# TrungMasterChef/CSWin-SimAM-UNet

Measured on AMD Instinct MI355X. Metric: images/sec at 512×512 bf16, 1/2/4/8 MI355X; Dice parity vs reference, higher is better.
Workload: dtype bf16; 1 GPU; CSWin-UNet train step 512x512 depth [1, 2, 9, 1] split [1, 2, 8, 8] +SimAM, AdamW; model=CSWinTransformer, params=23567980, global_batch=16, per_gpu_batch=16, img=512, parallelism=dp1, workload_key=cswin|d1,2,9,1|s1,2,8,8|simam|bf16|512|16

## Files before the change

cswin-simam-unet_amd/csrc/gemm_ws.hip:

```cpp
#include "common.hpp"

#include <type_traits>

namespace csu {
namespace {

enum { WS_PLAIN = 0, WS_RESID = 1, WS_LNBWD = 2, WS_RESID_LN = 3 };

struct WsLnF {
    const float* gamma;
    const float* beta;
    float eps;
    bf16* out;
    float* mean;
    float* rstd;
};

struct WsLn {
    const float* x;
    const float* gamma;
    const float* mean;
    const float* rstd;
    const float* dres;
    float* dx;
    bf16* dxb;
    float* part;
};

constexpr int WS_BM = 64;
constexpr bool WS_ROT = true;

constexpr int ws_unit(int ks, int nt, int umax = 16) {
    for (int u = umax; u > 1; --u)
        if (ks % u == 0 && nt * (ks / u) >= 2) return u;
    for (int u = umax; u > 1; --u)
        if (ks % u == 0) return u;
    return 1;
}
constexpr int ws_wn(int n) { return (n / 32) % 4 == 0 ? 4 : (n / 32) % 2 == 0 ? 2 : 1; }
constexpr int ws_tokens(int n) { return WS_BM * (4 / ws_wn(n)); }
#ifndef WS_NSPLIT
#define WS_NSPLIT 1
#endif
constexpr int ws_ns(int k, int n, int epi) {
    return WS_NSPLIT > 1 && epi == 0 && k <= 256 && ws_wn(n) == 4 && (n / 128) % WS_NSPLIT == 0 ? WS_NSPLIT : 1;
}

__device__ __forceinline__ bf16x8 e4m3x8_bf16(u32x2 w) {
    typedef __bf16 bf16x2v __attribute__((ext_vector_type(2)));
    const bf16x2v p0 = __builtin_amdgcn_cvt_scalef32_pk_bf16_fp8(w[0], 1.f, false);
    const bf16x2v p1 = __builtin_amdgcn_cvt_scalef32_pk_bf16_fp8(w[0], 1.f, true);
    const bf16x2v p2 = __builtin_amdgcn_cvt_scalef32_pk_bf16_fp8(w[1], 1.f, false);
    const bf16x2v p3 = __builtin_amdgcn_cvt_scalef32_pk_bf16_fp8(w[1], 1.f, true);
    return bf16x8{p0[0], p0[1], p1[0], p1[1], p2[0], p2[1], p3[0], p3[1]};
}

template <int K, int N, int EPI, typename TOUT, int NS = 1, int F8 = 0>
__global__ __launch_bounds__(256, ws_wn(N) < 4 || NS > 1 ? 2 : 1) void gemm_ws_kernel(long M, const bf16* __restrict__ X, int ldx,
                                                      const bf16* __restrict__ Wf, const float* __restrict__ bias,
                                                      const float* __restrict__ resid, TOUT* __restrict__ out,
                                                      WsLn ln = WsLn{}, WsLnF lnf = WsLnF{},
                                                      const float* __restrict__ wsc = nullptr) {
    static_assert(F8 == 0 || EPI != WS_LNBWD, "gemm_ws: e4m3 weights not with the LayerNorm-backward epilogue");
    constexpr int WN = ws_wn(N);
    constexpr int NT = N / (32 * WN * NS);
    static_assert(NT * 32 * WN * NS == N, "gemm_ws: N = 32 WN NT NS");
    static_assert(NS == 1 || EPI == WS_PLAIN || EPI == WS_RESID, "gemm_ws: the LayerNorm epilogues need all N features");
    static_assert(EPI != WS_LNBWD || WN == 4, "gemm_ws: the LayerNorm epilogue needs all C features in one token group");
    constexpr int KS = K / 16;
    constexpr int UK = ws_unit(KS, NT, NS > 1 ? 8 : 16);
    constexpr int CH = KS / UK;
    static_assert(CH * UK == KS, "unit size");
    constexpr int U = NT * CH;
    constexpr bool XREG = K <= 256;
    constexpr bool XLDS = !XREG || WN == 4;
    constexpr int XS = K + 8;
    constexpr int ES = 36;
    __shared__ __attribute__((aligned(16))) bf16 xs[XLDS ? WS_BM * XS : 8];
    __shared__ __attribute__((aligned(16))) float ep_all[4 * WS_BM * ES];

    const int lane = threadIdx.x & 63;
    const int wave = __builtin_amdgcn_readfirstlane(threadIdx.x >> 6);
    const int wn = wave % WN;
    const int r = lane & 31, h = lane >> 5;
    const long m0 = (long)blockIdx.x * ws_tokens(N) + WS_BM * (wave / WN);
    float* ep = ep_all + wave * WS_BM * ES;

    const int rot = WS_ROT ? (int)((blockIdx.x >> 3) % NT) : 0;
    const int tb = NS > 1 ? (int)blockIdx.y * NT : 0;
    auto tile_of = [&](int i) { return tb + (i + rot < NT ? i + rot : i + rot - NT); };
    using WFR = std::conditional_t<F8 != 0, u32x2, bf16x8>;
    WFR wf[2][UK];
    auto wload1 = [&](int u, int s) {
        const int nt = wn + WN * tile_of(u / CH), ks = (u % CH) * UK + s;
        if constexpr (F8 != 0)
            wf[u & 1][s] = *reinterpret_cast<const u32x2*>(reinterpret_cast<const uint8_t*>(Wf) +
                                                           ((long)(nt * KS + ks) * 64 + lane) * 8);
        else
            wf[u & 1][s] = *reinterpret_cast<const bf16x8*>(Wf + ((long)(nt * KS + ks) * 64 + lane) * 8);
    };
    auto wfrag = [&](const WFR& w) {
        if constexpr (F8 != 0) return e4m3x8_bf16(w);
        else return w;
    };
#pragma unroll
    for (int s = 0; s < UK; ++s) wload1(0, s);
    __builtin_amdgcn_sched_barrier(0);
    bf16x8 xf[XREG ? 2 : 1][XREG ? KS : 1];
    if constexpr (XLDS) {
        constexpr int PR = K / 8;
#pragma unroll
        for (int i = 0; i < WS_BM * PR / 256; ++i) {
            const int p = threadIdx.x + 256 * i, row = p / PR, c = 8 * (p % PR);
            bf16x8 v = *reinterpret_cast<const bf16x8*>(X + (m0 + row) * ldx + c);
            if constexpr (F8 == 2) {
                const f32x4 s0 = *reinterpret_cast<const f32x4*>(wsc + c), s1 = *reinterpret_cast<const f32x4*>(wsc + c + 4);
#pragma unroll
                for (int e = 0; e < 4; ++e) {
                    v[e] = (bf16)((float)v[e] * s0[e]);
                    v[4 + e] = (bf16)((float)v[4 + e] * s1[e]);
                }
            }
            *reinterpret_cast<bf16x8*>(xs + row * XS + c) = v;
        }
        __syncthreads();
        if constexpr (XREG) {
#pragma unroll
            for (int t = 0; t < 2; ++t)
#pragma unroll
                for (int s = 0; s < KS; ++s) xf[t][s] = *reinterpret_cast<const bf16x8*>(xs + (32 * t + r) * XS + 16 * s + 8 * h);
        }
    } else {
#pragma unroll
        for (int t = 0; t < 2; ++t)
#pragma unroll
            for (int s = 0; s < KS; ++s) {
                xf[t][s] = *reinterpret_cast<const bf16x8*>(X + (m0 + 32 * t + r) * ldx + 16 * s + 8 * h);
                if constexpr (F8 == 2) {
#pragma unroll
                    for (int e = 0; e < 8; ++e) xf[t][s][e] = (bf16)((float)xf[t][s][e] * wsc[16 * s + 8 * h + e]);
                }
            }
    }
    __builtin_amdgcn_sched_barrier(0);

    f32x16 a0 = f32x16{}, a1 = f32x16{};
    const auto rs_b = buf_rsrc(bias, bias ? (long)N * 4 : 0);
    constexpr bool BF = sizeof(TOUT) == 2;
    constexpr bool RES = EPI == WS_RESID || EPI == WS_RESID_LN;
    static_assert(EPI != WS_RESID_LN || !BF, "gemm_ws: the LayerNorm epilogue writes the fp32 residual stream");
    float bv[8], rv[8][4], sv[8];
    const auto rs_s = buf_rsrc(wsc, F8 == 1 ? (long)N * 4 : 0);
    f32x16 keep[EPI == WS_LNBWD ? NT : 1][2];
    float yk[EPI == WS_RESID_LN ? NT : 1][8][4];
    float lg[EPI == WS_RESID_LN ? NT : 1][4], lb[EPI == WS_RESID_LN ? NT : 1][4];
    if constexpr (EPI == WS_RESID_LN) {
        const int cc = 4 * (lane & 7);
#pragma unroll
        for (int i = 0; i < NT; ++i) {
            load4(lnf.gamma + 32 * (wn + WN * tile_of(i)) + cc, lg[i]);
            load4(lnf.beta + 32 * (wn + WN * tile_of(i)) + cc, lb[i]);
        }
    }
#pragma unroll
    for (int u = 0; u < U; ++u) {
        const int c = u % CH;
        if (EPI != WS_LNBWD && c == CH - 1) {
            const int n0 = 32 * (wn + WN * tile_of(u / CH));
            if constexpr (BF) {
                const int cc = 8 * (lane & 3);
                buf_ld4(rs_b, (unsigned)(n0 + cc) * 4, bv);
                buf_ld4(rs_b, (unsigned)(n0 + cc + 4) * 4, bv + 4);
                if constexpr (F8 == 1) {
                    buf_ld4(rs_s, (unsigned)(n0 + cc) * 4, sv);
                    buf_ld4(rs_s, (unsigned)(n0 + cc + 4) * 4, sv + 4);
                }
            } else {
                const int cc = 4 * (lane & 7);
                buf_ld4(rs_b, (unsigned)(n0 + cc) * 4, bv);
                if constexpr (F8 == 1) buf_ld4(rs_s, (unsigned)(n0 + cc) * 4, sv);
                if constexpr (RES) {
                    const auto rs_res = buf_rsrc(resid + m0 * N, (M - m0) * N * 4);
#pragma unroll
                    for (int q = 0; q < 8; ++q) buf_ld4(rs_res, (unsigned)((8 * q + (lane >> 3)) * N + n0 + cc) * 4, rv[q]);
                }
            }
        }
        __builtin_amdgcn_sched_barrier(0);
#pragma unroll
        for (int s = 0; s < UK; ++s) {
            if (u + 1 < U) wload1(u + 1, s);
            const int ks = c * UK + s;
            bf16x8 b0, b1;
            if constexpr (XREG) {
                b0 = xf[0][ks];
                b1 = xf[XREG ? 1 : 0][ks];
            } else {
                b0 = *reinterpret_cast<const bf16x8*>(xs + r * XS + 16 * ks + 8 * h);
                b1 = *reinterpret_cast<const bf16x8*>(xs + (32 + r) * XS + 16 * ks + 8 * h);
            }
            const bf16x8 wa = wfrag(wf[u & 1][s]);
            a0 = __builtin_amdgcn_mfma_f32_32x32x16_bf16(wa, b0, a0, 0, 0, 0);
            a1 = __builtin_amdgcn_mfma_f32_32x32x16_bf16(wa, b1, a1, 0, 0, 0);
            if (u + 1 < U) __builtin_amdgcn_sched_group_barrier(0x020, 1, 0);
            if constexpr (!XREG) __builtin_amdgcn_sched_group_barrier(0x100, 2, 0);
            __builtin_amdgcn_sched_group_barrier(0x008, 2, 0);
        }
        __builtin_amdgcn_sched_barrier(0);
        if (c != CH - 1) continue;
        if constexpr (EPI == WS_LNBWD) {
            keep[u / CH][0] = a0;
            keep[u / CH][1] = a1;
            a0 = f32x16{};
            a1 = f32x16{};
            continue;
        }
        const int nt = wn + WN * tile_of(u / CH);
#pragma unroll
        for (int t = 0; t < 2; ++t) {
            const f32x16& a = t ? a1 : a0;
#pragma unroll
            for (int g = 0; g < 4; ++g)
                *reinterpret_cast<f32x4*>(ep + (32 * t + r) * ES + 8 * g + 4 * h) =
                    f32x4{a[4 * g], a[4 * g + 1], a[4 * g + 2], a[4 * g + 3]};
        }
        asm volatile("" ::: "memory");
        const int n0 = 32 * nt;
        const auto rs_out = buf_rsrc(out + m0 * N, (M - m0) * N * (long)sizeof(TOUT));
        if constexpr (BF) {
            const int cc = 8 * (lane & 3);
#pragma unroll
            for (int q = 0; q < 4; ++q) {
                const int row = 16 * q + (lane >> 2);
                float v[8];
                load4(ep + row * ES + cc, v);
                load4(ep + row * ES + cc + 4, v + 4);
#pragma unroll
                for (int e = 0; e < 8; ++e) {
                    if constexpr (F8 == 1) v[e] *= sv[e];
                    v[e] += bv[e];
                }
                buf_st8bf(rs_out, (unsigned)(row * N + n0 + cc) * 2, v);
            }
        } else {
            const int cc = 4 * (lane & 7);
#pragma unroll
            for (int q = 0; q < 8; ++q) {
                const int row = 8 * q + (lane >> 3);
                float v[4];
                load4(ep + row * ES + cc, v);
#pragma unroll
                for (int e = 0; e < 4; ++e) {
                    if constexpr (F8 == 1) v[e] *= sv[e];
                    v[e] += bv[e];
                    if constexpr (RES) v[e] += rv[q][e];
                    if constexpr (EPI == WS_RESID_LN) yk[u / CH][q][e] = v[e];
                }
                buf_st4(rs_out, (unsigned)(row * N + n0 + cc) * 4, v);
            }
        }
        a0 = f32x16{};
        a1 = f32x16{};
        __builtin_amdgcn_sched_barrier(0);
    }
    if constexpr (EPI == WS_RESID_LN) {
        __shared__ float lnx[2][4][WS_BM];
        const int rq = lane >> 3, g0 = (wave / WN) * WN;
        float mu[8], rsd[8];
#pragma unroll
        for (int pass = 0; pass < 2; ++pass) {
#pragma unroll
            for (int q = 0; q < 8; ++q) {
                float a = 0.f;
#pragma unroll
                for (int i = 0; i < NT; ++i)
#pragma unroll
                    for (int e = 0; e < 4; ++e) {
                        const float d = pass ? yk[i][q][e] - mu[q] : yk[i][q][e];
                        a = pass ? fmaf(d, d, a) : a + d;
                    }
                a = sum8_dpp(a);
                if ((lane & 7) == 0) lnx[pass][wave][8 * q + rq] = a;
            }
            __syncthreads();
#pragma unroll
            for (int q = 0; q < 8; ++q) {
                float t = 0.f;
#pragma unroll
                for (int j = 0; j < WN; ++j) t += lnx[pass][g0 + j][8 * q + rq];
                if (pass) rsd[q] = rsqrtf(t * (1.f / N) + lnf.eps);
                else mu[q] = t * (1.f / N);
            }
        }
        const auto rs_ln = buf_rsrc(lnf.out + m0 * N, (M - m0) * N * 2);
        const int cc = 4 * (lane & 7);
#pragma unroll
        for (int i = 0; i < NT; ++i) {
            const int n0 = 32 * (wn + WN * tile_of(i));
#pragma unroll
            for (int q = 0; q < 8; ++q) {
                float o[4];
#pragma unroll
                for (int e = 0; e < 4; ++e) o[e] = (yk[i][q][e] - mu[q]) * rsd[q] * lg[i][e] + lb[i][e];
                buf_st4bf(rs_ln, (unsigned)((8 * q + rq) * N + n0 + cc) * 2, o);
            }
        }
        if (wn == 0 && (lane & 7) == 0) {
#pragma unroll
            for (int q = 0; q < 8; ++q) {
                lnf.mean[m0 + 8 * q + rq] = mu[q];
                lnf.rstd[m0 + 8 * q + rq] = rsd[q];
            }
        }
    }
    if constexpr (EPI == WS_LNBWD) {
        constexpr int C = N;
        const auto rs_x = buf_rsrc(ln.x + m0 * C, (M - m0) * C * 4);
        const auto rs_r = buf_rsrc(ln.dres ? ln.dres + m0 * C : nullptr, ln.dres ? (M - m0) * C * 4 : 0);
        float mu[2], rs[2];
#pragma unroll
        for (int t = 0; t < 2; ++t) {
            mu[t] = ln.mean[m0 + 32 * t + r];
            rs[t] = ln.rstd[m0 + 32 * t + r];
        }
        float xh[NT][2][16], gam[NT][16];
        float rv2[NT][2][16];
#pragma unroll
        for (int i = 0; i < NT; ++i) {
            const int n0 = 32 * (wn + WN * tile_of(i));
#pragma unroll
            for (int g = 0; g < 4; ++g) {
                load4(ln.gamma + n0 + 8 * g + 4 * h, gam[i] + 4 * g);
#pragma unroll
                for (int t = 0; t < 2; ++t) {
                    const unsigned off = (unsigned)((32 * t + r) * C + n0 + 8 * g + 4 * h) * 4;
                    buf_ld4(rs_x, off, xh[i][t] + 4 * g);
                    buf_ld4(rs_r, off, rv2[i][t] + 4 * g);
                }
            }
        }
        float s1[2] = {0.f, 0.f}, s2[2] = {0.f, 0.f};
        float dgc[NT][16], dbc[NT][16];
#pragma unroll
        for (int i = 0; i < NT; ++i)
#pragma unroll
            for (int j = 0; j < 16; ++j) {
                dgc[i][j] = 0.f;
                dbc[i][j] = 0.f;
#pragma unroll
                for (int t = 0; t < 2; ++t) {
                    const float dh = keep[i][t][j];
                    const float x_h = (xh[i][t][j] - mu[t]) * rs[t];
                    xh[i][t][j] = x_h;
                    const float gg = dh * gam[i][j];
                    s1[t] += gg;
                    s2[t] += gg * x_h;
                    dgc[i][j] += dh * x_h;
                    dbc[i][j] += dh;
                }
            }
        float* lnx = ep_all;
#pragma unroll
        for (int t = 0; t < 2; ++t) {
            s1[t] += __shfl_xor(s1[t], 32, 64);
            s2[t] += __shfl_xor(s2[t], 32, 64);
            if (h == 0) {
                lnx[(wave * 2 + 0) * 64 + 32 * t + r] = s1[t];
                lnx[(wave * 2 + 1) * 64 + 32 * t + r] = s2[t];
            }
        }
        __syncthreads();
        float S1[2], S2[2];
#pragma unroll
        for (int t = 0; t < 2; ++t) {
            S1[t] = S2[t] = 0.f;
#pragma unroll
            for (int w = 0; w < 4; ++w) {
                S1[t] += lnx[(w * 2 + 0) * 64 + 32 * t + r];
                S2[t] += lnx[(w * 2 + 1) * 64 + 32 * t + r];
            }
            S1[t] *= 1.f / C;
            S2[t] *= 1.f / C;
        }
        const auto rs_dx = buf_rsrc(ln.dx + m0 * C, (M - m0) * C * 4);
        const auto rs_dxb = buf_rsrc(ln.dxb + m0 * C, (M - m0) * C * 2);
#pragma unroll
        for (int i = 0; i < NT; ++i) {
            const int n0 = 32 * (wn + WN * tile_of(i));
#pragma unroll
            for (int t = 0; t < 2; ++t)
#pragma unroll
                for (int g = 0; g < 4; ++g) {
                    float o[4];
#pragma unroll
                    for (int e = 0; e < 4; ++e) {
                        const int j = 4 * g + e;
                        o[e] = rs[t] * (keep[i][t][j] * gam[i][j] - S1[t] - xh[i][t][j] * S2[t]) + rv2[i][t][j];
                    }
                    const unsigned off = (unsigned)((32 * t + r) * C + n0 + 8 * g + 4 * h);
                    buf_st4(rs_dx, off * 4, o);
                    buf_st4bf(rs_dxb, off * 2, o);
                }
        }
#pragma unroll
        for (int o = 1; o < 32; o <<= 1)
#pragma unroll
            for (int i = 0; i < NT; ++i)
#pragma unroll
                for (int j = 0; j < 16; ++j) {
                    dgc[i][j] += __shfl_xor(dgc[i][j], o, 64);
                    dbc[i][j] += __shfl_xor(dbc[i][j], o, 64);
                }
        if (r == 0) {
            float* prow = ln.part + (size_t)blockIdx.x * 2 * C;
#pragma unroll
            for (int i = 0; i < NT; ++i) {
                const int n0 = 32 * (wn + WN * tile_of(i));
#pragma unroll
                for (int g = 0; g < 4; ++g) {
                    store4(prow + n0 + 8 * g + 4 * h, dgc[i] + 4 * g);
                    store4(prow + C + n0 + 8 * g + 4 * h, dbc[i] + 4 * g);
                }
            }
        }
    }
}

template <int K, int N, int EPI, typename TOUT, int F8 = 0>
int ws_launch(long M, const bf16* X, int ldx, const bf16* Wf, const float* bias, const float* resid, void* out,
              hipStream_t st, const WsLn& ln = WsLn{}, const WsLnF& lnf = WsLnF{}, const float* wsc = nullptr) {
    constexpr int NS = F8 ? 1 : ws_ns(K, N, EPI);
    gemm_ws_kernel<K, N, EPI, TOUT, NS, F8><<<dim3((unsigned)(M / ws_tokens(N)), NS), 256, 0, st>>>(
        M, X, ldx, Wf, bias, resid, (TOUT*)out, ln, lnf, wsc);
    return check_launch("gemm_ws");
}

#define WS_SHAPES(X_) X_(128, 384) X_(256, 768) X_(384, 128) X_(768, 256) X_(128, 128) X_(256, 256) \
    X_(64, 192) X_(64, 64)

}

int gemm_ws_supported(long M, int N, int K, int resid, int out_dtype) {
    if (M < ws_tokens(N) || M % ws_tokens(N) || M > (1L << 30)) return 0;
    if (resid && out_dtype != CSU_F32) return 0;
    if (out_dtype != CSU_F32 && out_dtype != CSU_BF16) return 0;
#define WS_HAS(KK, NN) if (K == KK && N == NN) return 1;
    WS_SHAPES(WS_HAS)
#undef WS_HAS
    return 0;
}

int gemm_ws_run(long M, int N, int K, const bf16* X, int ldx, const bf16* Wf, const float* bias, const float* resid,
                int out_dtype, void* out, hipStream_t st) {
#define WS_GO(KK, NN)                                                                                             \
    if (K == KK && N == NN) {                                                                                     \
        if (resid) return ws_launch<KK, NN, WS_RESID, float>(M, X, ldx, Wf, bias, resid, out, st);          \
        if (out_dtype == CSU_F32) return ws_launch<KK, NN, WS_PLAIN, float>(M, X, ldx, Wf, bias, nullptr, out, st); \
        return ws_launch<KK, NN, WS_PLAIN, bf16>(M, X, ldx, Wf, bias, nullptr, out, st);                    \
    }
    WS_SHAPES(WS_GO)
#undef WS_GO
    return fail(CSU_E_ARG, "gemm_ws: shape not instantiated");
}

int gemm_ws_e4m3_run(long M, int N, int K, const bf16* X, int ldx, const uint8_t* Wq, const float* wsc, int mode,
                     const float* bias, const float* resid, int out_dtype, void* out, hipStream_t st) {
    const bf16* W = reinterpret_cast<const bf16*>(Wq);
#define WS_GO8(KK, NN, MODE)                                                                                      \
    if (K == KK && N == NN && mode == MODE) {                                                                     \
        if (resid) return ws_launch<KK, NN, WS_RESID, float, MODE>(M, X, ldx, W, bias, resid, out, st, {}, {}, wsc); \
        if (out_dtype == CSU_F32)                                                                                 \
            return ws_launch<KK, NN, WS_PLAIN, float, MODE>(M, X, ldx, W, bias, nullptr, out, st, {}, {}, wsc);   \
        return ws_launch<KK, NN, WS_PLAIN, bf16, MODE>(M, X, ldx, W, bias, nullptr, out, st, {}, {}, wsc);        \
    }
#define WS_GO8B(KK, NN) WS_GO8(KK, NN, 1) WS_GO8(KK, NN, 2)
    WS_SHAPES(WS_GO8B)
#undef WS_GO8B
#undef WS_GO8
    return fail(CSU_E_ARG, "gemm_ws_e4m3: shape not instantiated");
}

int gemm_ws_ln_supported(long M, int N, int K) {
    if (M < ws_tokens(N) || M % ws_tokens(N) || M > (1L << 30)) return 0;
    return K == N && (N == 64 || N == 128 || N == 256);
}

int gemm_ws_ln_run(long M, int N, const bf16* X, int ldx, const bf16* Wf, const float* bias, const float* resid, float* out,
                   const WsLnF& lnf, hipStream_t st, const float* wsc = nullptr) {
    if (wsc) {
        if (N == 64) return ws_launch<64, 64, WS_RESID_LN, float, 1>(M, X, ldx, Wf, bias, resid, out, st, WsLn{}, lnf, wsc);
        if (N == 128) return ws_launch<128, 128, WS_RESID_LN, float, 1>(M, X, ldx, Wf, bias, resid, out, st, WsLn{}, lnf, wsc);
        if (N == 256) return ws_launch<256, 256, WS_RESID_LN, float, 1>(M, X, ldx, Wf, bias, resid, out, st, WsLn{}, lnf, wsc);
        return fail(CSU_E_ARG, "gemm_ws_ln_e4m3: shape not instantiated");
    }
    if (N == 64) return ws_launch<64, 64, WS_RESID_LN, float>(M, X, ldx, Wf, bias, resid, out, st, WsLn{}, lnf);
    if (N == 128) return ws_launch<128, 128, WS_RESID_LN, float>(M, X, ldx, Wf, bias, resid, out, st, WsLn{}, lnf);
    if (N == 256) return ws_launch<256, 256, WS_RESID_LN, float>(M, X, ldx, Wf, bias, resid, out, st, WsLn{}, lnf);
    return fail(CSU_E_ARG, "gemm_ws_ln: shape not instantiated");
}

int gemm_ws_lnbwd_supported(long M, int N, int K) {
    if (M < WS_BM || M % WS_BM || M > (1L << 30)) return 0;
    return (K == 384 && N == 128) || (K == 768 && N == 256);
}

int gemm_ws_lnbwd_run(long M, int N, int K, const bf16* dy, const bf16* Wtf, const WsLn& ln, hipStream_t st) {
    if (K == 384 && N == 128) return ws_launch<384, 128, WS_LNBWD, float>(M, dy, K, Wtf, nullptr, nullptr, nullptr, st, ln);
    if (K == 768 && N == 256) return ws_launch<768, 256, WS_LNBWD, float>(M, dy, K, Wtf, nullptr, nullptr, nullptr, st, ln);
    return fail(CSU_E_ARG, "gemm_ws_lnbwd: shape not instantiated");
}

__global__ __launch_bounds__(256) void frag_layout_kernel(const csu_frag_item* __restrict__ items, int count) {
    const long g = (long)blockIdx.x * 256 + threadIdx.x;
    int lo = 0, hi = count - 1;
    while (lo < hi) {
        const int mid = (lo + hi + 1) >> 1;
        if (items[mid].chunk0 <= g) lo = mid; else hi = mid - 1;
    }
    const csu_frag_item it = items[lo];
    const long q = g - it.chunk0;
    const int qc = it.cols / 8;
    if (q < 0 || q >= (long)it.rows * qc) return;
    const int n = (int)(q / qc), k8 = (int)(q % qc);
    const long dst = (((long)(n >> 5) * (it.cols >> 4) + (k8 >> 1)) * 64 + (n & 31) + 32 * (k8 & 1)) * 8;
    *reinterpret_cast<u32x4*>((bf16*)it.dst + dst) = *reinterpret_cast<const u32x4*>((const bf16*)it.src + q * 8);
}

__device__ __forceinline__ long frag8_chunk(int row, int c8, int cols) {
    return ((long)(row >> 5) * (cols >> 4) + (c8 >> 1)) * 64 + (row & 31) + 32 * (c8 & 1);
}
__global__ __launch_bounds__(256) void frag8_layout_kernel(const csu_frag8_item* __restrict__ items, int count) {
    const long g = (long)blockIdx.x * 256 + threadIdx.x;
    int lo = 0, hi = count - 1;
    while (lo < hi) {
        const int mid = (lo + hi + 1) >> 1;
        if (items[mid].block0 <= g) lo = mid; else hi = mid - 1;
    }
    const csu_frag8_item it = items[lo];
    const long b = g - it.block0;
    const int kb = it.K / 8;
    if (b < 0 || b >= (long)(it.N / 8) * kb) return;
    const int n0 = 8 * (int)(b / kb), k0 = 8 * (int)(b % kb);
    const uint8_t* src = reinterpret_cast<const uint8_t*>(it.src);
    u32x2 v[8];
#pragma unroll
    for (int i = 0; i < 8; ++i) v[i] = *reinterpret_cast<const u32x2*>(src + (long)(n0 + i) * it.K + k0);
    u32x2* dst = reinterpret_cast<u32x2*>(it.dst);
    if (!it.transpose) {
#pragma unroll
        for (int i = 0; i < 8; ++i) dst[frag8_chunk(n0 + i, k0 >> 3, it.K)] = v[i];
    } else {
#pragma unroll
        for (int j = 0; j < 8; ++j) {
            unsigned lo4 = 0, hi4 = 0;
#pragma unroll
            for (int i = 0; i < 4; ++i) {
                lo4 |= ((v[i][j >> 2] >> (8 * (j & 3))) & 0xffu) << (8 * i);
                hi4 |= ((v[4 + i][j >> 2] >> (8 * (j & 3))) & 0xffu) << (8 * i);
            }
            dst[frag8_chunk(k0 + j, n0 >> 3, it.N)] = u32x2{lo4, hi4};
        }
    }
}

}

using namespace csu;

extern "C" int csu_gemm_ws_supported(long M, int N, int K, int resid, int out_dtype) {
    return gemm_ws_supported(M, N, K, resid, out_dtype);
}

extern "C" int csu_gemm_ws(long M, int N, int K, const void* x, int ldx, const void* w_frag, const float* bias,
                           const float* resid, int out_dtype, void* out, void* stream) {
    if (!x || !w_frag || !out) return fail(CSU_E_ARG, "gemm_ws: null pointer");
    if (!gemm_ws_supported(M, N, K, resid != nullptr, out_dtype)) return fail(CSU_E_ARG, "gemm_ws: unsupported shape");
// ... 63 lines not shown
```

cswin-simam-unet_amd/csu/ops.py:

```python
from __future__ import annotations

import ctypes
import os
import threading
import weakref
from typing import List, Optional, Sequence, Tuple

import torch

from . import _lib
from ._lib import CSU_BF16, CSU_F32, CsuError, check, dtype_code, lib, ptr, require_device, stream_ptr
from .ledger import esize, launch as _launch, prec_of


def _stripe_fwd_work(geom, B, esize):
    L = geom.reso * geom.reso
    nb = len(geom.branches)
    hs, ws, _ = geom.branches[0]
    N = hs * ws
    nbytes = B * L * (3 * geom.C + geom.C) * esize + nb * B * geom.heads * L * 4
    flops = B * L * nb * geom.heads * 4 * N * geom.head_dim + 18 * B * L * geom.C
    return nbytes, flops


# ... 2122 lines not shown
            self._layout_frag8(dev)
            return self.deq
        if self.lay_count:
            _launch("quant_e4m3", lambda: lib().csu_e4m3_layout_batch(ptr(self.lay_items), self.lay_count, self.lay_words,
                                                                     stream_ptr(dev)), 0, self.lay_words * 8)
        self._layout_frag8(dev)
        return self.deq

    def _layout_frag8(self, dev):
        if self.frag8_count and FP8_WS:
            n = self.frag8_blocks * 64
            _launch("quant_e4m3", lambda: lib().csu_frag8_layout_batch(ptr(self.frag8_items), self.frag8_count,
                                                                      self.frag8_blocks, stream_ptr(dev)), 0, 2 * n)


_ACTIVE_CACHE: Optional[CastCache] = None
_ACTIVE_FP8: Optional[Fp8Weights] = None


def set_cast_cache(cache: Optional[CastCache], fp8: Optional[Fp8Weights] = None):
    global _ACTIVE_CACHE, _ACTIVE_FP8
    _ACTIVE_CACHE = cache
    _ACTIVE_FP8 = fp8


def fp8_gemm(aq: torch.Tensor, sa: torch.Tensor, wq: torch.Tensor, sw: torch.Tensor,
             bias: Optional[torch.Tensor] = None) -> torch.Tensor:
    require_device(aq, wq)
    M, K = aq.shape
    N = wq.shape[0]
    if wq.shape[1] != K or sa.numel() != M or sw.numel() != N or aq.dtype != torch.uint8 or wq.dtype != torch.uint8:
        raise ValueError("fp8_gemm: shape / dtype mismatch")
    aq, wq, sa, sw = aq.contiguous(), wq.contiguous(), sa.float().contiguous(), sw.float().contiguous()
    b = None if bias is None else bias.detach().float().contiguous()
    out = torch.empty(M, N, dtype=torch.bfloat16, device=aq.device)
    _launch("fp8_gemm", lambda: lib().csu_fp8_gemm(M, N, K, ptr(aq), ptr(sa), ptr(wq), ptr(sw), ptr(b), ptr(out),
                                                   stream_ptr(aq.device)),
            2 * M * N * K, M * K + N * K + M * N * 2 + (M + N) * 4, prec="fp8")
    return out


def dequant_e4m3_rows(q: torch.Tensor, scale: torch.Tensor) -> torch.Tensor:
    require_device(q)
    rows, cols = q.shape
    out = torch.empty(rows, cols, dtype=torch.bfloat16, device=q.device)
    _launch("dequant_e4m3", lambda: lib().csu_dequant_e4m3_rows(rows, cols, ptr(q), ptr(scale), ptr(out),
                                                                stream_ptr(q.device)),
            0, rows * cols * 3 + rows * 4, prec="fp8")
    return out


def layer_norm_fp8(x: torch.Tensor, weight: torch.Tensor, bias: torch.Tensor, eps: float = 1e-5, dq: bool = False):
    require_device(x, weight, bias)
    x = x.contiguous()
    C = x.shape[-1]
    rows = x.numel() // C
    w = weight.detach().float().contiguous()
    b = bias.detach().float().contiguous()
    q = torch.empty(rows, C, dtype=torch.uint8, device=x.device)
    s = torch.empty(rows, dtype=torch.float32, device=x.device)
    mean = torch.empty(rows, dtype=torch.float32, device=x.device)
    rstd = torch.empty(rows, dtype=torch.float32, device=x.device)
    ydq = torch.empty(rows, C, dtype=torch.bfloat16, device=x.device) if dq else None
    _launch("layernorm_fwd_fp8", lambda: lib().csu_layernorm_fwd_fp8_dq(rows, C, float(eps), dtype_code(x), ptr(x),
                                                                        ptr(w), ptr(b), ptr(q), ptr(s), ptr(ydq),
                                                                        ptr(mean), ptr(rstd), stream_ptr(x.device)),
            10 * rows * C, rows * C * (esize(x) + 1 + (2 if dq else 0)) + rows * 12, prec=prec_of(x))
    return (q, s, mean, rstd, ydq) if dq else (q, s, mean, rstd)


class _LnLinearFp8Fn(torch.autograd.Function):

    @staticmethod
    def forward(ctx, x, gamma, beta, weight, bias, eps: float, wq, ws, wt):
        x = x.contiguous()
        C = x.shape[-1]
        hq, hs, mean, rstd, hdq = layer_norm_fp8(x, gamma, beta, eps, dq=True)
        y = fp8_gemm(hq, hs, wq, ws, bias).view(*x.shape[:-1], wq.shape[0])
        ctx.save_for_backward(x, gamma.detach().float().contiguous(), mean, rstd, hdq, wt)
        ctx.params = (gamma, beta)
        ctx.pdtypes = (gamma.dtype, beta.dtype)
        ctx.lin = (weight, bias)
        ctx.lmeta = (weight.dtype, None if bias is None else bias.dtype, C)
        _note_use(ctx, gamma, beta, weight, bias)
        return x.view_as(x), y

    @staticmethod
    def backward(ctx, dres, dy):
        x, g, mean, rstd, h, wt = ctx.saved_tensors
        wdt, bdt, C = ctx.lmeta
        dh = dw = db = None
        if dy is not None:
            N = dy.shape[-1]
            dy2 = _bf16_of(dy).reshape(-1, N).contiguous()
            dh = gemm(dy2, wt, False, torch.bfloat16).view(x.shape)
            need_w, need_b = ctx.needs_input_grad[3], bdt is not None and ctx.needs_input_grad[4]
            if need_w or need_b:
                dwf, dbf = wgrad_maybe_side(dy2, h, wdt if need_w else None, bdt if need_b else None, params=ctx.lin)
                dw = dwf.to(wdt) if need_w else None
                db = dbf.to(bdt) if need_b else None
        dx, dg, dbeta = _ln_fork_backward(ctx, x, g, mean, rstd, dres, dh)
        return dx, dg, dbeta, dw, db, None, None, None, None


class _LnLinearWsFn(torch.autograd.Function):

    @staticmethod
    def forward(ctx, x, gamma, beta, weight, bias, eps: float, wf, wtf, pre):
        x = x.contiguous()
        C = x.shape[-1]
        rows = x.numel() // C
        g = gamma.detach().float().contiguous()
        if pre is not None:
            h1, mean, rstd = pre[3].view(x.shape), pre[4], pre[5]
        else:
            b = beta.detach().float().contiguous()
            h1 = torch.empty(x.shape, dtype=torch.bfloat16, device=x.device)
            mean = torch.empty(rows, dtype=torch.float32, device=x.device)
            rstd = torch.empty(rows, dtype=torch.float32, device=x.device)
            _launch("layernorm_fwd", lambda: lib().csu_layernorm_fwd(rows, C, float(eps), dtype_code(x), ptr(x), ptr(g),
                                                                     ptr(b), CSU_BF16, ptr(h1), ptr(mean), ptr(rstd),
                                                                     stream_ptr(x.device)),
                    8 * rows * C, rows * C * (4 + 2) + rows * 8, prec="f32")
        N = weight.shape[0]
        h2 = h1.view(rows, C)
        y = gemm_ws(h2, wf, N, torch.bfloat16, bias=None if bias is None else bias.detach().float().contiguous())
        ctx.save_for_backward(x, g, mean, rstd, h2, wtf)
        ctx.params = (gamma, beta)
        ctx.pdtypes = (gamma.dtype, beta.dtype)
        ctx.lin = (weight, bias)
        ctx.lmeta = (weight.dtype, None if bias is None else bias.dtype)
        _note_use(ctx, gamma, beta, weight, bias)
        return x.view_as(x), y.view(*x.shape[:-1], N)

    @staticmethod
    def backward(ctx, dres, dy):
        x, g, mean, rstd, h, wtf = ctx.saved_tensors
        wdt, bdt = ctx.lmeta
        C = x.shape[-1]
        rows = x.numel() // C
        if dy is None:
            dx, dg, dbeta = _ln_fork_backward(ctx, x, g, mean, rstd, dres, None)
            return dx, dg, dbeta, None, None, None, None, None, None
        N = dy.shape[-1]
        dy2 = _bf16_of(dy).reshape(-1, N).contiguous()
        dres_k = dres.float().contiguous() if dres is not None else None
        dx = torch.empty_like(x)
        dxb = torch.empty(x.shape, dtype=torch.bfloat16, device=x.device)
        nblk = rows // 64
        work = torch.empty(nblk * 2 * C, dtype=torch.float32, device=x.device)
        _launch("gemm", lambda: lib().csu_gemm_ws_lnbwd(rows, C, N, ptr(dy2), ptr(wtf), ptr(x), ptr(g), ptr(mean), ptr(rstd),
                                                       ptr(dres_k), ptr(dx), ptr(dxb), ptr(work), stream_ptr(x.device)),
                2 * rows * N * C + 12 * rows * C,
                rows * N * 2 + N * C * 2 + rows * C * (4 + (4 if dres_k is not None else 0) + 4 + 2) + rows * 8,
                prec="bf16", tag=f"{rows}x{C}x{N}:lnbwd:ws")
        dgb = _grad_dest(ctx.params)
        if dgb is None:
            dgb = torch.empty(2 * C, dtype=torch.float32, device=x.device)
        if not _ln_params(ctx, rows, C, work, dgb, nblocks=nblk):
            it = (_lib.LnParamItem * 1)()
            it[0].workspace, it[0].dgamma, it[0].dbeta = work.data_ptr(), dgb.data_ptr(), dgb.data_ptr() + C * 4
            it[0].rows, it[0].C, it[0].nblocks = rows, C, nblk
            _launch("layernorm_bwd", lambda: lib().csu_layernorm_param_reduce_batch(it, 1, stream_ptr(x.device)),
                    0, work.numel() * 4 + 2 * C * 4)
        dw = db = None
        need_w, need_b = ctx.needs_input_grad[3], bdt is not None and ctx.needs_input_grad[4]
        if need_w or need_b:
            dwf, dbf = wgrad_maybe_side(dy2, h, wdt if need_w else None, bdt if need_b else None, params=ctx.lin)
            dw = dwf.to(wdt) if need_w else None
            db = dbf.to(bdt) if need_b else None
        dx._csu_bf16 = dxb
        return dx, dgb[:C].to(ctx.pdtypes[0]), dgb[C:].to(ctx.pdtypes[1]), dw, db, None, None, None, None


FUSE_LN_QKV = False


def ln_linear_ws(x: torch.Tensor, ln: torch.nn.LayerNorm, lin: torch.nn.Linear):
    if not (FUSE_LN_QKV and USE_GEMM_WS and x.is_cuda and x.dtype == torch.float32 and _ACTIVE_CACHE is not None
            and (_ACTIVE_FP8 is None or not FP8_WS)):
        return None
    N, K = lin.weight.shape
    if x.shape[-1] != K or ln.weight.numel() != K or ln.weight.dtype != torch.float32:
        return None
    wf, wtf = _ACTIVE_CACHE.get_frag(lin.weight), _ACTIVE_CACHE.get_frag_t(lin.weight)
    M = x.numel() // K
    if wf is None or wtf is None or not _ws_ok(M, N, K, torch.bfloat16) or not lib().csu_gemm_ws_lnbwd_supported(M, K, N):
        return None
    pre = _ln_pre(x, ln.weight, ln.bias, ln.eps, torch.bfloat16)
    with torch.autocast("cuda", enabled=False):
        return _LnLinearWsFn.apply(x, ln.weight, ln.bias, lin.weight, lin.bias, ln.eps, wf, wtf, pre)


FP8_QKV = os.environ.get("CSU_FP8_QKV", "0") != "0"


def ln_linear_fp8(x: torch.Tensor, ln: torch.nn.LayerNorm, lin: torch.nn.Linear):
    if _ACTIVE_FP8 is None or not x.is_cuda or not FP8_QKV:
        return None
    got = _ACTIVE_FP8.lookup(lin.weight)
    N, K = lin.weight.shape
    if got is None or N % 64 or K % 64 or K > 512:
        return None
    wc = _ACTIVE_CACHE.get(lin.weight, torch.bfloat16) if _ACTIVE_CACHE is not None else None
    if wc is None:
        return None
    wt = _weight_t(lin.weight, wc)
    with torch.autocast("cuda", enabled=False):
        return _LnLinearFp8Fn.apply(x, ln.weight, ln.bias, lin.weight, lin.bias, ln.eps, got[0], got[1], wt)


def linear(x: torch.Tensor, weight: torch.Tensor, bias: Optional[torch.Tensor] = None,
           out_dtype: Optional[torch.dtype] = None) -> torch.Tensor:
    if x.is_cuda and torch.is_autocast_enabled("cuda"):
        cd = torch.get_autocast_dtype("cuda")
    else:
        cd = torch.promote_types(x.dtype, weight.dtype)
    wc = _ACTIVE_CACHE.get(weight, cd) if _ACTIVE_CACHE is not None else None
    with torch.autocast("cuda", enabled=False):
        return _LinearFn.apply(x, weight, bias, cd, wc, out_dtype)


def _conv_geom(B, H, W, C, N, KH, KW, stride, pad):
    g = _lib.ConvGeom()
    g.B, g.H, g.W, g.C, g.N, g.KH, g.KW, g.stride, g.pad = B, H, W, C, N, KH, KW, stride, pad
    g.OH, g.OW = (H + 2 * pad - KH) // stride + 1, (W + 2 * pad - KW) // stride + 1
    return g


def _conv_wgrad(g, x, dy, dt, c_real=None, out=None):
    L = lib()
    cr = g.C if c_real is None else c_real
    if out is None:
        out = torch.empty(g.N * g.KH * g.KW * cr + g.N, dtype=torch.float32, device=x.device)
    n = L.csu_conv2d_wgrad_workspace(ctypes.byref(g))
    work = torch.empty(max(n, 16), dtype=torch.uint8, device=x.device)
    _launch("conv_wgrad", lambda: L.csu_conv2d_wgrad_oihw(ctypes.byref(g), dt, ptr(x), ptr(dy), cr, ptr(out), ptr(work),
                                                          n, stream_ptr(x.device)),
            2 * g.B * g.OH * g.OW * g.N * g.KH * g.KW * g.C,
            (g.B * g.H * g.W * g.C + g.B * g.OH * g.OW * g.N) * x.element_size() + out.numel() * 4, prec=prec_of(x))
    k = g.N * g.KH * g.KW * cr
    return out[:k].view(g.N, cr, g.KH, g.KW), out[k:]


def _pad_channels(C: int) -> int:
    return (C + 7) // 8 * 8 if (C % 8 and PAD_CHANNELS) else C


def _conv_ws(op: int, g, t: torch.Tensor):
    n = lib().csu_conv2d_workspace(op, ctypes.byref(g), dtype_code(t))
    if not n:
        return None, 0
    return torch.empty(n, dtype=torch.uint8, device=t.device), n


class _Conv2dFn(torch.autograd.Function):
    @staticmethod
    def forward(ctx, x, weight, bias, stride: int, pad: int, cd):
        require_device(x, weight)
        B, H, W, C = x.shape
        N, Cw, KH, KW = weight.shape
        if Cw != C:
            raise ValueError(f"conv2d: input has {C} channels, weight expects {Cw}")
        cp = _pad_channels(C)
        if cp != C:
            xn = x.permute(0, 3, 1, 2)
            if cd == torch.bfloat16 and x.dtype == torch.float32 and xn.is_contiguous():
                xc = torch.empty(B, H, W, cp, dtype=cd, device=x.device)
                _launch("pack_nhwc", lambda: lib().csu_pack_nhwc_bf16(B, C, H, W, cp, ptr(xn), ptr(xc), stream_ptr(x.device)),
                        0, x.numel() * 4 + xc.numel() * 2, prec="f32")
            else:
                xc = torch.zeros(B, H, W, cp, dtype=cd, device=x.device)
                xc[..., :C] = x
            cached = _ACTIVE_CACHE.get_conv(weight, cd) if _ACTIVE_CACHE is not None else None
            if cached is not None and cached[0].shape[-1] == cp:
                w_ohwi = cached[0]
            else:
                w_ohwi = torch.nn.functional.pad(weight.detach().permute(0, 2, 3, 1).to(cd), (0, cp - C)).contiguous()
            cached = None
        else:
            xc = (x if x.dtype == cd else x.to(cd)).contiguous()
            cached = _ACTIVE_CACHE.get_conv(weight, cd) if _ACTIVE_CACHE is not None else None
            w_ohwi = cached[0] if cached else weight.detach().permute(0, 2, 3, 1).to(cd).contiguous()
        g = _conv_geom(B, H, W, cp, N, KH, KW, stride, pad)
        y = torch.empty(B, g.OH, g.OW, N, dtype=cd, device=x.device)
        bf = None if bias is None else bias.detach().float().contiguous()
        ws, nws = _conv_ws(0, g, xc)
        _launch("conv_fwd", lambda: lib().csu_conv2d_fwd_ws(ctypes.byref(g), dtype_code(xc), ptr(xc), ptr(w_ohwi), ptr(bf),
                                                            ptr(y), ptr(ws), nws, stream_ptr(x.device)),
                2 * y.numel() * KH * KW * cp, (xc.numel() + w_ohwi.numel() + y.numel()) * xc.element_size(), prec=prec_of(xc))
        ctx.save_for_backward(xc, weight)
        ctx.w_ihwo = cached[1] if cached else None
        ctx.bias = bias
        _note_use(ctx, weight, bias)
        ctx.conf = (stride, pad, cd, x.dtype, bias is not None, None if bias is None else bias.dtype)
        return y

    @staticmethod
    def backward(ctx, dy):
        xc, weight = ctx.saved_tensors
        stride, pad, cd, xdt, has_b, bdt = ctx.conf
        B, H, W, cp = xc.shape
        N, C, KH, KW = weight.shape
        g = _conv_geom(B, H, W, cp, N, KH, KW, stride, pad)
        dy = dy.to(cd).contiguous()
        dx = None
        if ctx.needs_input_grad[0]:
            if cp != C:
                w_ihwo = torch.nn.functional.pad(weight.detach().permute(1, 2, 3, 0).to(cd), (0, 0, 0, 0, 0, 0, 0, cp - C))
                w_ihwo = w_ihwo.contiguous()
            else:
                w_ihwo = ctx.w_ihwo if ctx.w_ihwo is not None else weight.detach().permute(1, 2, 3, 0).to(cd).contiguous()
            dx = torch.empty(B, H, W, cp, dtype=cd, device=dy.device)
            ws, nws = _conv_ws(1, g, dy)
            _launch("conv_dgrad", lambda: lib().csu_conv2d_dgrad_ws(ctypes.byref(g), dtype_code(dy), ptr(dy), ptr(w_ihwo),
                                                                    None, ptr(dx), ptr(ws), nws, stream_ptr(dy.device)),
                    2 * dy.numel() * KH * KW * cp, (dy.numel() + w_ihwo.numel() + dx.numel()) * dy.element_size(),
                    prec=prec_of(dy))
            if cp != C:
                dx = dx[..., :C]
            if dx.dtype != xdt:
                dx = dx.to(xdt)

        dest = None
        if has_b and weight.dtype == torch.float32 and bdt == torch.float32:
            dest = _grad_dest((weight, ctx.bias))
            if dest is not None and dest.numel() != N * KH * KW * C + N:
                dest = None
# ... 148 lines not shown
```

Baseline: 1570 images/sec.

## Restructure LayerNorm-backward GEMM epilogue via LDS row phase and enable LN-QKV fusion

The LayerNorm-backward epilogue of the weight-stationary GEMM now writes each accumulated dh tile to shared memory instead of holding all tiles in registers. A row-wise phase then computes the normalization backward with DPP/readlane reductions, prefetching x and the residual gradient during the MFMA loop. Column partials for dgamma/dbeta are reduced through the reused token panel. Occupancy is raised to 2 for C<=128, and the fused LN+QKV path is enabled by default via an environment flag. This lowers register pressure and turns on a previously disabled fusion, at the cost of extra LDS traffic and synchronisation.

```diff
diff --git a/cswin-simam-unet_amd/csrc/gemm_ws.hip b/cswin-simam-unet_amd/csrc/gemm_ws.hip
--- a/cswin-simam-unet_amd/csrc/gemm_ws.hip
+++ b/cswin-simam-unet_amd/csrc/gemm_ws.hip
@@ -55,8 +55,27 @@
     return bf16x8{p0[0], p0[1], p1[0], p1[1], p2[0], p2[1], p3[0], p3[1]};
 }
 
+template <int LPR> __device__ __forceinline__ float ln_row_sum(float x) {
+    x = sum8_dpp(x);
+    x += dppf<0x128>(x);
+    x = xsum16(x);
+    if constexpr (LPR == 64) x = xsum32(x);
+    return x;
+}
+template <int RPI> __device__ __forceinline__ float ln_row_val(float v, int i, int lane) {
+    const int b = __builtin_bit_cast(int, v);
+    if constexpr (RPI == 1) return __builtin_bit_cast(float, __builtin_amdgcn_readlane(b, i));
+    else {
+        const int lo = __builtin_amdgcn_readlane(b, 2 * i), hi = __builtin_amdgcn_readlane(b, 2 * i + 1);
+        return __builtin_bit_cast(float, lane < 32 ? lo : hi);
+    }
+}
+
+constexpr int ws_ep_floats(int n, int epi) { return epi == WS_LNBWD ? WS_BM * (n + 4) / 2 : 4 * WS_BM * 36; }
+constexpr int ws_occ(int n, int epi, int ns) { return ws_wn(n) < 4 || ns > 1 || (epi == WS_LNBWD && n <= 128) ? 2 : 1; }
+
 template <int K, int N, int EPI, typename TOUT, int NS = 1, int F8 = 0>
-__global__ __launch_bounds__(256, ws_wn(N) < 4 || NS > 1 ? 2 : 1) void gemm_ws_kernel(long M, const bf16* __restrict__ X, int ldx,
+__global__ __launch_bounds__(256, ws_occ(N, EPI, NS)) void gemm_ws_kernel(long M, const bf16* __restrict__ X, int ldx,
                                                       const bf16* __restrict__ Wf, const float* __restrict__ bias,
                                                       const float* __restrict__ resid, TOUT* __restrict__ out,
                                                       WsLn ln = WsLn{}, WsLnF lnf = WsLnF{},
@@ -77,14 +96,15 @@
     constexpr int XS = K + 8;
     constexpr int ES = 36;
     __shared__ __attribute__((aligned(16))) bf16 xs[XLDS ? WS_BM * XS : 8];
-    __shared__ __attribute__((aligned(16))) float ep_all[4 * WS_BM * ES];
+    static_assert(ES == 36, "ws_ep_floats");
+    __shared__ __attribute__((aligned(16))) float ep_all[ws_ep_floats(N, EPI)];
 
     const int lane = threadIdx.x & 63;
     const int wave = __builtin_amdgcn_readfirstlane(threadIdx.x >> 6);
     const int wn = wave % WN;
     const int r = lane & 31, h = lane >> 5;
     const long m0 = (long)blockIdx.x * ws_tokens(N) + WS_BM * (wave / WN);
-    float* ep = ep_all + wave * WS_BM * ES;
+    float* ep = ep_all + (EPI == WS_LNBWD ? 0 : wave * WS_BM * ES);
 
     const int rot = WS_ROT ? (int)((blockIdx.x >> 3) % NT) : 0;
     const int tb = NS > 1 ? (int)blockIdx.y * NT : 0;
@@ -151,7 +171,18 @@
     static_assert(EPI != WS_RESID_LN || !BF, "gemm_ws: the LayerNorm epilogue writes the fp32 residual stream");
     float bv[8], rv[8][4], sv[8];
     const auto rs_s = buf_rsrc(wsc, F8 == 1 ? (long)N * 4 : 0);
-    f32x16 keep[EPI == WS_LNBWD ? NT : 1][2];
+    constexpr bool LNB = EPI == WS_LNBWD;
+    constexpr int LN_LPR = LNB ? N / 4 : 64, LN_RPI = 64 / LN_LPR, LN_NI = 16 / LN_RPI;
+    constexpr int LN_PPU = (2 * LN_NI + U - 1) / U;
+    constexpr int LN_DS = N + 4;
+    static_assert(!LNB || (LN_LPR == 32 || LN_LPR == 64), "gemm_ws: the row phase holds C = 128 or 256");
+    static_assert(!LNB || WS_BM * LN_DS * 2 <= (int)sizeof(ep_all), "gemm_ws: the dh tile must fit the epilogue region");
+    static_assert(!LNB || (XLDS && 8 * N * 4 <= (int)sizeof(xs)), "gemm_ws: the column partials reuse the token panel");
+    bf16* dht = reinterpret_cast<bf16*>(ep_all);
+    const int ln_c0 = 4 * (lane % LN_LPR);
+    float px[LNB ? LN_NI : 1][4], pr[LNB ? LN_NI : 1][4], ln_gw[4], ln_mu = 0.f, ln_rs = 0.f;
+    const auto rs_lx = buf_rsrc(LNB ? ln.x + m0 * N : nullptr, LNB ? (M - m0) * N * 4 : 0);
+    const auto rs_lr = buf_rsrc(LNB && ln.dres ? ln.dres + m0 * N : nullptr, LNB && ln.dres ? (M - m0) * N * 4 : 0);
     float yk[EPI == WS_RESID_LN ? NT : 1][8][4];
     float lg[EPI == WS_RESID_LN ? NT : 1][4], lb[EPI == WS_RESID_LN ? NT : 1][4];
     if constexpr (EPI == WS_RESID_LN) {
@@ -165,6 +196,22 @@
 #pragma unroll
     for (int u = 0; u < U; ++u) {
         const int c = u % CH;
+        if constexpr (LNB) {
+            if (u == 0) {
+                load4(ln.gamma + ln_c0, ln_gw);
+                ln_mu = ln.mean[m0 + 16 * wave + (lane & 15)];
+                ln_rs = ln.rstd[m0 + 16 * wave + (lane & 15)];
+            }
+#pragma unroll
+            for (int j = 0; j < LN_PPU; ++j) {
+                const int p = u * LN_PPU + j, i = p >> 1;
+                if (p < 2 * LN_NI) {
+                    const unsigned off = (unsigned)((16 * wave + LN_RPI * i + lane / LN_LPR) * N + ln_c0) * 4;
+                    if (p & 1) buf_ld4(rs_lr, off, pr[i]);
+                    else buf_ld4(rs_lx, off, px[i]);
+                }
+            }
+        }
         if (EPI != WS_LNBWD && c == CH - 1) {
             const int n0 = 32 * (wn + WN * tile_of(u / CH));
             if constexpr (BF) {
@@ -209,8 +256,16 @@
         __builtin_amdgcn_sched_barrier(0);
         if (c != CH - 1) continue;
         if constexpr (EPI == WS_LNBWD) {
-            keep[u / CH][0] = a0;
-            keep[u / CH][1] = a1;
+            const int n0 = 32 * (wn + WN * tile_of(u / CH));
+#pragma unroll
+            for (int t = 0; t < 2; ++t) {
+                const f32x16& a = t ? a1 : a0;
+#pragma unroll
+                for (int g = 0; g < 4; ++g) {
+                    const float v[4] = {a[4 * g], a[4 * g + 1], a[4 * g + 2], a[4 * g + 3]};
+                    store4(dht + (32 * t + r) * LN_DS + n0 + 8 * g + 4 * h, v);
+                }
+            }
             a0 = f32x16{};
             a1 = f32x16{};
             continue;
@@ -314,114 +369,55 @@
         }
     }
     if constexpr (EPI == WS_LNBWD) {
-        constexpr int C = N;
-        const auto rs_x = buf_rsrc(ln.x + m0 * C, (M - m0) * C * 4);
-        const auto rs_r = buf_rsrc(ln.dres ? ln.dres + m0 * C : nullptr, ln.dres ? (M - m0) * C * 4 : 0);
-        float mu[2], rs[2];
-#pragma unroll
-        for (int t = 0; t < 2; ++t) {
-            mu[t] = ln.mean[m0 + 32 * t + r];
-            rs[t] = ln.rstd[m0 + 32 * t + r];
-        }
-        float xh[NT][2][16], gam[NT][16];
-        float rv2[NT][2][16];
-#pragma unroll
-        for (int i = 0; i < NT; ++i) {
-            const int n0 = 32 * (wn + WN * tile_of(i));
-#pragma unroll
-            for (int g = 0; g < 4; ++g) {
-                load4(ln.gamma + n0 + 8 * g + 4 * h, gam[i] + 4 * g);
-#pragma unroll
-                for (int t = 0; t < 2; ++t) {
-                    const unsigned off = (unsigned)((32 * t + r) * C + n0 + 8 * g + 4 * h) * 4;
-                    buf_ld4(rs_x, off, xh[i][t] + 4 * g);
-                    buf_ld4(rs_r, off, rv2[i][t] + 4 * g);
-                }
-            }
-        }
-        float s1[2] = {0.f, 0.f}, s2[2] = {0.f, 0.f};
-        float dgc[NT][16], dbc[NT][16];
-#pragma unroll
-        for (int i = 0; i < NT; ++i)
-#pragma unroll
-            for (int j = 0; j < 16; ++j) {
-                dgc[i][j] = 0.f;
-                dbc[i][j] = 0.f;
-#pragma unroll
-                for (int t = 0; t < 2; ++t) {
-                    const float dh = keep[i][t][j];
-                    const float x_h = (xh[i][t][j] - mu[t]) * rs[t];
-                    xh[i][t][j] = x_h;
-                    const float gg = dh * gam[i][j];
-                    s1[t] += gg;
-                    s2[t] += gg * x_h;
-                    dgc[i][j] += dh * x_h;
-                    dbc[i][j] += dh;
-                }
-            }
-        float* lnx = ep_all;
-#pragma unroll
-        for (int t = 0; t < 2; ++t) {
-            s1[t] += __shfl_xor(s1[t], 32, 64);
-            s2[t] += __shfl_xor(s2[t], 32, 64);
-            if (h == 0) {
-                lnx[(wave * 2 + 0) * 64 + 32 * t + r] = s1[t];
-                lnx[(wave * 2 + 1) * 64 + 32 * t + r] = s2[t];
-            }
-        }
         __syncthreads();
-        float S1[2], S2[2];
-#pragma unroll
-        for (int t = 0; t < 2; ++t) {
-            S1[t] = S2[t] = 0.f;
-#pragma unroll
-            for (int w = 0; w < 4; ++w) {
-                S1[t] += lnx[(w * 2 + 0) * 64 + 32 * t + r];
-                S2[t] += lnx[(w * 2 + 1) * 64 + 32 * t + r];
-            }
-            S1[t] *= 1.f / C;
-            S2[t] *= 1.f / C;
-        }
-        const auto rs_dx = buf_rsrc(ln.dx + m0 * C, (M - m0) * C * 4);
-        const auto rs_dxb = buf_rsrc(ln.dxb + m0 * C, (M - m0) * C * 2);
-#pragma unroll
-        for (int i = 0; i < NT; ++i) {
-            const int n0 = 32 * (wn + WN * tile_of(i));
-#pragma unroll
-            for (int t = 0; t < 2; ++t)
-#pragma unroll
-                for (int g = 0; g < 4; ++g) {
-                    float o[4];
-#pragma unroll
-                    for (int e = 0; e < 4; ++e) {
-                        const int j = 4 * g + e;
-                        o[e] = rs[t] * (keep[i][t][j] * gam[i][j] - S1[t] - xh[i][t][j] * S2[t]) + rv2[i][t][j];
-                    }
-                    const unsigned off = (unsigned)((32 * t + r) * C + n0 + 8 * g + 4 * h);
-                    buf_st4(rs_dx, off * 4, o);
-                    buf_st4bf(rs_dxb, off * 2, o);
-                }
-        }
-#pragma unroll
-        for (int o = 1; o < 32; o <<= 1)
-#pragma unroll
-            for (int i = 0; i < NT; ++i)
-#pragma unroll
-                for (int j = 0; j < 16; ++j) {
-                    dgc[i][j] += __shfl_xor(dgc[i][j], o, 64);
-                    dbc[i][j] += __shfl_xor(dbc[i][j], o, 64);
-                }
-        if (r == 0) {
-            float* prow = ln.part + (size_t)blockIdx.x * 2 * C;
-#pragma unroll
-            for (int i = 0; i < NT; ++i) {
-                const int n0 = 32 * (wn + WN * tile_of(i));
-#pragma unroll
-                for (int g = 0; g < 4; ++g) {
-                    store4(prow + n0 + 8 * g + 4 * h, dgc[i] + 4 * g);
-                    store4(prow + C + n0 + 8 * g + 4 * h, dbc[i] + 4 * g);
-                }
-            }
+        const auto rs_dx = buf_rsrc(ln.dx + m0 * N, (M - m0) * N * 4);
+        const auto rs_dxb = buf_rsrc(ln.dxb + m0 * N, (M - m0) * N * 2);
+        float dg[4] = {0.f, 0.f, 0.f, 0.f}, db[4] = {0.f, 0.f, 0.f, 0.f};
+#pragma unroll
+        for (int i = 0; i < LN_NI; ++i) {
+            const int q = LN_RPI * i + lane / LN_LPR;
+            float dh[4], xh[4], gg[4], o[4];
+            load4(dht + (16 * wave + q) * LN_DS + ln_c0, dh);
+            const float mu = ln_row_val<LN_RPI>(ln_mu, i, lane), rs = ln_row_val<LN_RPI>(ln_rs, i, lane);
+            float s1 = 0.f, s2 = 0.f;
+#pragma unroll
+            for (int e = 0; e < 4; ++e) {
+                xh[e] = (px[i][e] - mu) * rs;
+                gg[e] = dh[e] * ln_gw[e];
+                s1 += gg[e];
+                s2 += gg[e] * xh[e];
+                dg[e] += dh[e] * xh[e];
+                db[e] += dh[e];
+            }
+            s1 = ln_row_sum<LN_LPR>(s1) / N;
+            s2 = ln_row_sum<LN_LPR>(s2) / N;
+#pragma unroll
+            for (int e = 0; e < 4; ++e) o[e] = rs * (gg[e] - s1 - xh[e] * s2) + pr[i][e];
+            const unsigned off = (unsigned)((16 * wave + q) * N + ln_c0);
+            buf_st4(rs_dx, off * 4, o);
+            buf_st4bf(rs_dxb, off * 2, o);
+        }
+        float* red = reinterpret_cast<float*>(xs);
+        if constexpr (LN_RPI == 2) {
+#pragma unroll
+            for (int e = 0; e < 4; ++e) {
+                dg[e] += __shfl_xor(dg[e], 32, 64);
+                db[e] += __shfl_xor(db[e], 32, 64);
+            }
+        }
+        if (lane < LN_LPR) {
+            store4(red + (wave * 2 + 0) * N + ln_c0, dg);
+            store4(red + (wave * 2 + 1) * N + ln_c0, db);
+        }
+        __syncthreads();
+        float* prow = ln.part + (size_t)blockIdx.x * 2 * N;
+#pragma unroll
+        for (int i = threadIdx.x; i < 2 * N; i += 256) {
+            const int k = i / N, c = i % N;
+            float s = 0.f;
+#pragma unroll
+            for (int w = 0; w < 4; ++w) s += red[(w * 2 + k) * N + c];
+            prow[i] = s;
         }
     }
 }
diff --git a/cswin-simam-unet_amd/csu/ops.py b/cswin-simam-unet_amd/csu/ops.py
--- a/cswin-simam-unet_amd/csu/ops.py
+++ b/cswin-simam-unet_amd/csu/ops.py
@@ -2298,7 +2298,8 @@
         _launch("gemm", lambda: lib().csu_gemm_ws_lnbwd(rows, C, N, ptr(dy2), ptr(wtf), ptr(x), ptr(g), ptr(mean), ptr(rstd),
                                                        ptr(dres_k), ptr(dx), ptr(dxb), ptr(work), stream_ptr(x.device)),
                 2 * rows * N * C + 12 * rows * C,
-                rows * N * 2 + N * C * 2 + rows * C * (4 + (4 if dres_k is not None else 0) + 4 + 2) + rows * 8,
+                rows * N * 2 + N * C * 2 + rows * C * (4 + (4 if dres_k is not None else 0)) + C * 4 + rows * 8
+                + rows * C * (4 + 2) + work.numel() * 4,
                 prec="bf16", tag=f"{rows}x{C}x{N}:lnbwd:ws")
         dgb = _grad_dest(ctx.params)
         if dgb is None:
@@ -2319,7 +2320,7 @@
         return dx, dgb[:C].to(ctx.pdtypes[0]), dgb[C:].to(ctx.pdtypes[1]), dw, db, None, None, None, None
 
 
-FUSE_LN_QKV = False
+FUSE_LN_QKV = os.environ.get("CSU_FUSE_LN_QKV", "1") != "0"
 
 
 def ln_linear_ws(x: torch.Tensor, ln: torch.nn.LayerNorm, lin: torch.nn.Linear):
```

Result: faster. 1603 images/sec, median of 6 (+2.1%).
